# syghmon/bridges-with-reinforcement-learning

Hardware: AMD Instinct MI355X
Metric: env-steps/sec (vectorised assembly_gym, tower_height=4) (higher is better)
Workload: dtype f64

## Files before the change

__graft_entry__.py:

```python
import os
import subprocess
import sys

ROOT = os.path.dirname(os.path.abspath(__file__))
PKG = os.path.join(ROOT, "bridges-with-reinforcement-learning_amd")
for p in (ROOT, PKG):
    if p not in sys.path:
        sys.path.insert(0, p)

HIPCC = os.environ.get("HIPCC", "/opt/rocm/bin/hipcc")
HIP_FLAGS = ["--offload-arch=gfx950", "-O3", "-ffp-contract=off", "-fPIC", "-shared", "-std=c++17"]


def build():
    from bridges_hip import abi
    src = os.path.join(PKG, "csrc", "api.hip")
    out = os.path.join(PKG, "bridges_hip", "libbridges_hip.so")
    want = abi.source_hash()
    if abi.library_stamp(out) != want:
        tmp = out + ".tmp"
        subprocess.check_call([HIPCC, *HIP_FLAGS, f'-DBRIDGES_SRC_HASH="{want}"', src, "-o", tmp])
        os.replace(tmp, out)
        assert abi.library_stamp(out) == want, "the built library does not carry its source stamp"
    oracle_mk = os.path.join(ROOT, "oracle", "Makefile")
    if os.path.exists(oracle_mk):
        subprocess.check_call(["make", "-s", "-C", os.path.join(ROOT, "oracle")])
    import bridges_hip
    L = abi.lib()
    for sym in abi.EXPORTED_SYMBOLS:
        getattr(L, sym)


def smoke():
    import numpy as np
    import torch
    from bridges_hip.shapes import load_urdf
    from bridges_hip.vec_env import VecAssemblyGym
    from oracle.env import OracleGym, OracleLockstep, bridge_setup, policy_draw

    assert torch.cuda.is_available(), "smoke() needs cuda:0"
    E, seed = 8, 5
    setup = bridge_setup(num_stories=2)
    vec = VecAssemblyGym(E, [load_urdf("shapes/trapezoid.urdf")], setup["obstacles"], setup["targets"],
                         max_steps=10, seed=seed)
    oracles = [OracleLockstep(OracleGym(**setup, max_steps=10)) for _ in range(E)]
    counters = [0] * E
    for it in range(6):
        vec.select_random()
        outs = []
        for e, o in enumerate(oracles):
            def pick(nv, e=e):
                r = policy_draw(seed, e, counters[e]) % nv
                counters[e] += 1
                return r
            outs.append(o.lockstep(pick))
        vec.step()
        torch.cuda.synchronize()
        fl = {k: v.cpu().numpy() for k, v in vec.flags().items()}
        for e, out in enumerate(outs):
            if out["valid_step"]:
                assert bool(fl["stable_frozen"][e]) == out["stable_frozen"]
                assert bool(fl["stable_unfrozen"][e]) == out["stable_unfrozen"]
                assert bool(fl["done"][e]) == out["done"]
        off = vec.cand_offset.cpu().numpy()
        mask = vec.cand_mask.cpu().numpy()
        for e, o in enumerate(oracles):
            A = len(o.cand["actions"])
            assert np.array_equal(mask[off[e]:off[e] + A].astype(bool), o.cand["mask"])
    print("smoke ok: 6 lock-steps x 8 envs bit-identical to the oracle")


if __name__ == "__main__":
    {"build": build, "smoke": smoke}[sys.argv[1] if len(sys.argv) > 1 else "build"]()
```

bridges-with-reinforcement-learning_amd/csrc/api.hip:

```cpp
#include <hip/hip_runtime.h>
#include <cstdio>
#include <cstdlib>
#include <cstring>
#include <new>

#include "env_kernels.hip"
#include "ops_kernels.hip"
#include "dqn_kernels.hip"
#include "mlp_kernels.hip"
#include "conv_kernels.hip"
#include "conv_train_kernels.hip"
#include "replay_kernels.hip"
#include "hindsight_kernels.hip"
#include "fork_kernels.hip"
#include "beam_kernels.hip"
#include "soft_target_kernels.hip"
#include "munchausen_kernels.hip"

using namespace bridges;

static thread_local char g_err[512] = "";

static int fail_hip(hipError_t e, const char* what) {
    snprintf(g_err, sizeof(g_err), "%s: %s", what, hipGetErrorString(e));
    return BRIDGES_E_HIP;
}
static int fail_arg(const char* what) {
    snprintf(g_err, sizeof(g_err), "bad argument: %s", what);
    return BRIDGES_E_ARG;
}
static int fail_arg(const char* who, const char* what) {
    snprintf(g_err, sizeof(g_err), "bad argument: %s: %s", who, what);
    return BRIDGES_E_ARG;
}
#define HIP_TRY(x)                                        \
    do {                                                  \
        hipError_t e_ = (x);                              \
        if (e_ != hipSuccess) return fail_hip(e_, #x);    \
    } while (0)

template <typename... P, typename... A>
static int launch(const char* name, void (*k)(P...), dim3 grid, dim3 block, size_t lds, void* stream, A... a) {
    hipLaunchKernelGGL(k, grid, block, lds, (hipStream_t)stream, a...);
    const hipError_t e = hipGetLastError();
    return e == hipSuccess ? BRIDGES_OK : fail_hip(e, name);
}

template <typename... T>
static bool aligned(uintptr_t bytes, const T*... p) {
    return ((((uintptr_t)p) | ... | (uintptr_t)0) & (bytes - 1)) == 0;
}

static int64_t ceil_div(int64_t a, int64_t b) { return (a + b - 1) / b; }

static int64_t clamp_grid(int64_t blocks, int64_t limit) {
    if (blocks < 1) blocks = 1;
    return blocks > limit ? limit : blocks;
}

static int grid_for_waves(int64_t n_items) { return (int)clamp_grid(ceil_div(n_items, 4), 2048); }

static int up2_splits(int64_t tiles, int* tps) {
    int per = (int)((tiles + 255) / 256);
    if (per < 1) per = 1;
    *tps = per;
    return (int)((tiles + per - 1) / per);
}

typedef void (*c3_fn)(const float*, const float*, const float*, const float*, const float*, float*, int, int, int, int, int);
template <int W, int CH>
static c3_fn c3_epilogue(int mode) {
    if (mode == C3_EPI_BIAS_RELU) return k_c3<W, CH, C3_EPI_BIAS_RELU>;
    if (mode == C3_EPI_MASK) return k_c3<W, CH, C3_EPI_MASK>;
    return k_c3<W, CH, C3_EPI_RAW>;
}
template <int W>
static c3_fn c3_kernel(int c_in, int mode) { return c_in <= 4 ? c3_epilogue<W, 4>(mode) : c3_epilogue<W, 16>(mode); }

struct bridges_gate {
    hipEvent_t last;
};

struct bridges_env {
    bridges_gate* gate;
    hipEvent_t raster_done;
    DevCtx ctx;
    TaskTable* tt_dev;
    int32_t* h_total;
    int max_blocks;
    int max_faces;
    hipEvent_t* ev_start;
    hipEvent_t* ev_stop;
    int ev_cap, ev_used;
    bool has_tasks;
    bridges_task_buffers tasks;
    const float* fixed_reward_map;
    const double* fixed_reward_prefix;
    bridges_task_family family;
    const uint64_t* family_thr;
};

static void clear_family(bridges_env* env) {
    memset(&env->family, 0, sizeof(env->family));
    env->family_thr = nullptr;
}

static long long candidate_estimate(const bridges_env* env) {
    long long est = (long long)(*(volatile int32_t*)env->h_total);
    if (est < env->ctx.E) est = env->ctx.E;
    return est + est / 32 + 64;
}

extern "C" {

const char* bridges_last_error(void) { return g_err; }

#ifndef BRIDGES_SRC_HASH
#define BRIDGES_SRC_HASH "unstamped"
#endif
const char* bridges_source_hash(void) { return "BRIDGES_SRC_HASH=" BRIDGES_SRC_HASH; }

int bridges_device_count(void) {
    int n = 0;
    if (hipGetDeviceCount(&n) != hipSuccess) return 0;
    return n;
}

int bridges_env_create(const bridges_task* t, const bridges_env_buffers* buf, bridges_env** out) {
    if (!t || !buf || !out) return fail_arg("null");
    if (t->n_envs <= 0) return fail_arg("n_envs");
    if (t->max_blocks <= 0 || t->max_blocks > BRIDGES_MAX_BLOCKS) return fail_arg("max_blocks > BRIDGES_MAX_BLOCKS");
    if (t->n_shapes <= 0 || t->n_shapes > 8) return fail_arg("n_shapes");
    if (t->n_groups <= 0 || t->n_groups > BRIDGES_MAX_GROUPS) return fail_arg("n_groups");
    if (t->n_ground < 0 || t->n_ground > 32 || t->n_offsets <= 0 || t->n_offsets > 8) return fail_arg("n_ground/n_offsets");
    if (t->n_targets < 0 || t->n_targets > BRIDGES_MAX_TARGETS) return fail_arg("n_targets");
    if (t->a_max <= 0) return fail_arg("a_max");
    if (t->img_size != 0 && (t->img_size < 2 || t->img_size > BRIDGES_IMG)) return fail_arg("img_size must be 0 (= 64) or 2..64");
    if (t->debug != 0) return fail_arg("debug must be 0");
    if (!buf->reward_prefix) return fail_arg("reward_prefix (float64 row prefix sums of reward_map) not given");
    if (buf->lp_ws_stride < (int64_t)BRIDGES_LP_WS_DOUBLES) return fail_arg("lp_ws_stride < BRIDGES_LP_WS_DOUBLES");
    static_assert(BRIDGES_LP_WS_DOUBLES == WARM_WS_DOUBLES, "header and device code disagree on the persistent tableau size");
    static_assert(BRIDGES_LP_SNAP_DOUBLES == WARM_HDR_DOUBLES + WARM_HALF, "header and device code disagree on the snapshot size");
    if (buf->lp_snap && buf->lp_snap_stride < (int64_t)BRIDGES_LP_SNAP_DOUBLES) return fail_arg("lp_snap_stride < BRIDGES_LP_SNAP_DOUBLES");
    for (int g = 0; g < t->n_groups; ++g) {
        if (t->group_shape[g] < 0 || t->group_shape[g] >= t->n_shapes) return fail_arg("group_shape");
        if (t->group_face[g] < 0 || t->group_face[g] >= t->shapes[t->group_shape[g]].nv) return fail_arg("group_face");
    }
    for (int s = 0; s < t->n_shapes; ++s)
        if (t->shapes[s].nv < 3 || t->shapes[s].nv > BRIDGES_MAX_VERTS) return fail_arg("shape nv");
    int ndev = 0;
    if (hipGetDeviceCount(&ndev) != hipSuccess || ndev == 0) {
        snprintf(g_err, sizeof(g_err), "no HIP device");
        return BRIDGES_E_NODEV;
    }
    bridges_env* env = new (std::nothrow) bridges_env();
    if (!env) return fail_arg("oom");
    TaskTable* host = new (std::nothrow) TaskTable();
    if (!host) { delete env; return fail_arg("oom"); }
    memset(host, 0, sizeof(TaskTable));
    memcpy(host->shapes, t->shapes, sizeof(bridges_shape) * t->n_shapes);
    memcpy(host->x_ground, t->x_ground, sizeof(double) * t->n_ground);
    memcpy(host->offsets, t->offsets, sizeof(double) * t->n_offsets);
    const int img = t->img_size ? t->img_size : IMG;
    for (int i = 0; i < IMG; ++i) {
        host->grid_x[i] = t->grid_x[i < img ? i : img - 1];
        host->grid_y[i] = t->grid_y[i < img ? i : img - 1];
    }
    hipError_t e = hipMalloc((void**)&env->tt_dev, sizeof(TaskTable));
    if (e == hipSuccess) e = hipMemcpy(env->tt_dev, host, sizeof(TaskTable), hipMemcpyHostToDevice);
    delete host;
    if (e != hipSuccess) { delete env; return fail_hip(e, "task table upload"); }
    DevCtx& c = env->ctx;
    memset(&c, 0, sizeof(c));
    c.b = *buf;
    c.tt = env->tt_dev;
    c.E = t->n_envs; c.K = t->max_blocks; c.max_steps = t->max_steps; c.a_max = t->a_max;
    c.n_groups = t->n_groups; c.n_ground = t->n_ground; c.n_offsets = t->n_offsets; c.n_targets = t->n_targets;
    memcpy(c.group_shape, t->group_shape, sizeof(c.group_shape));
    memcpy(c.group_face, t->group_face, sizeof(c.group_face));
    c.mu = t->mu; c.density = t->density; c.floor_hw = t->floor_half_width; c.floor_depth = t->floor_depth;
    c.xlim0 = t->xlim[0]; c.xlim1 = t->xlim[1]; c.ylim0 = t->ylim[0]; c.ylim1 = t->ylim[1];
    memcpy(c.targets, t->targets, sizeof(c.targets));
    c.seed = t->seed;
    c.debug = t->debug;
    c.env_id_base = t->env_id_base;
    c.n_shapes = t->n_shapes;
    c.img = img;
    env->ev_start = env->ev_stop = nullptr;
    env->ev_cap = env->ev_used = 0;
    env->gate = nullptr;
    env->raster_done = nullptr;
    env->has_tasks = false;
    memset(&env->tasks, 0, sizeof(env->tasks));
    clear_family(env);
    env->fixed_reward_map = buf->reward_map;
    env->fixed_reward_prefix = buf->reward_prefix;
    e = hipHostMalloc((void**)&env->h_total, sizeof(int32_t), hipHostMallocMapped | hipHostMallocCoherent);
    if (e == hipSuccess) e = hipHostGetDevicePointer((void**)&c.h_total, env->h_total, 0);
    if (e != hipSuccess) { (void)hipFree(env->tt_dev); delete env; return fail_hip(e, "hipHostMalloc"); }
    *env->h_total = t->n_envs * 64;
    env->max_blocks = 1 << 22;
    env->max_faces = 0;
    for (int g = 0; g < t->n_groups; ++g) {
        const int nv = t->shapes[t->group_shape[g]].nv;
        if (nv > env->max_faces) env->max_faces = nv;
    }
    *out = env;
    return BRIDGES_OK;
}

static void free_events(bridges_env* env) {
    for (int i = 0; i < env->ev_cap; ++i) {
        (void)hipEventDestroy(env->ev_start[i]);
        (void)hipEventDestroy(env->ev_stop[i]);
    }
    delete[] env->ev_start;
    delete[] env->ev_stop;
    env->ev_start = env->ev_stop = nullptr;
    env->ev_cap = env->ev_used = 0;
}

int bridges_env_destroy(bridges_env* env) {
    if (!env) return BRIDGES_OK;
    free_events(env);
    if (env->raster_done) (void)hipEventDestroy(env->raster_done);
    (void)hipFree(env->tt_dev);
    (void)hipHostFree(env->h_total);
    delete env;
    return BRIDGES_OK;
}

int bridges_gate_create(bridges_gate** out) {
    if (!out) return fail_arg("gate_create");
    bridges_gate* g = new (std::nothrow) bridges_gate();
    if (!g) return fail_arg("oom");
    g->last = nullptr;
    *out = g;
    return BRIDGES_OK;
}

int bridges_gate_destroy(bridges_gate* gate) {
    delete gate;
    return BRIDGES_OK;
}

int bridges_env_set_gate(bridges_env* env, bridges_gate* gate) {
    if (!env) return fail_arg("set_gate");
    if (gate && !env->raster_done) HIP_TRY(hipEventCreateWithFlags(&env->raster_done, hipEventDisableTiming));
    env->gate = gate;
    return BRIDGES_OK;
}

int bridges_env_timing_begin(bridges_env* env, int32_t max_launches) {
    if (!env || max_launches <= 0 || max_launches > (1 << 16)) return fail_arg("timing_begin");
    free_events(env);
    env->ev_start = new (std::nothrow) hipEvent_t[max_launches];
    env->ev_stop = new (std::nothrow) hipEvent_t[max_launches];
    if (!env->ev_start || !env->ev_stop) {
        delete[] env->ev_start;
        delete[] env->ev_stop;
        env->ev_start = env->ev_stop = nullptr;
        return fail_arg("oom");
    }
    for (int i = 0; i < max_launches; ++i) {
        HIP_TRY(hipEventCreate(&env->ev_start[i]));
        HIP_TRY(hipEventCreate(&env->ev_stop[i]));
        env->ev_cap = i + 1;
    }
    env->ev_used = 0;
    return BRIDGES_OK;
}

int bridges_env_timing_end(bridges_env* env, double* raster_ms_total, int32_t* n_launches) {
    if (!env || !raster_ms_total || !n_launches) return fail_arg("timing_end");
    double total = 0.0;
    for (int i = 0; i < env->ev_used; ++i) {
        HIP_TRY(hipEventSynchronize(env->ev_stop[i]));
        float ms = 0.f;
        HIP_TRY(hipEventElapsedTime(&ms, env->ev_start[i], env->ev_stop[i]));
        total += ms;
    }
    *raster_ms_total = total;
    *n_launches = env->ev_used;
    free_events(env);
    return BRIDGES_OK;
}

static int refresh(bridges_env* env, hipStream_t s, int after_step) {
    const DevCtx& c = env->ctx;
    if (int rc = launch("k_scan", k_scan, dim3(1), dim3(SCAN_THREADS), 0, s, c, after_step)) return rc;
    if (int rc = launch("k_enumerate", k_enumerate, dim3(c.E), dim3(WAVE), 0, s, c)) return rc;
    const long long items_est = candidate_estimate(env) + c.E;
    long long rblocks = ceil_div(items_est, 4);
    if (rblocks > env->max_blocks) rblocks = env->max_blocks;
    const bool timed = env->ev_cap > 0 && env->ev_used < env->ev_cap;
    if (env->gate && env->gate->last) HIP_TRY(hipStreamWaitEvent(s, env->gate->last, 0));
    if (timed) HIP_TRY(hipEventRecord(env->ev_start[env->ev_used], s));
    if (!env->has_tasks) {
        if (int rc = launch("k_raster", env->max_faces <= 4 ? k_raster<4> : k_raster<MAXV>, dim3((unsigned)rblocks), dim3(256), 0, s, c))
            return rc;
    } else if (env->tasks.n_obstacles == 0) {
        if (int rc = launch("k_raster (per-env tables)", env->max_faces <= 4 ? k_raster<4, true> : k_raster<MAXV, true>,
                            dim3((unsigned)rblocks), dim3(256), 0, s, c))
            return rc;
    } else if (int rc = launch("k_raster (per-env tables and obstacles)", env->max_faces <= 4 ? k_raster<4, true, const uint64_t*> : k_raster<MAXV, true, const uint64_t*>,
                               dim3((unsigned)rblocks), dim3(256), 0, s, c, (const uint64_t*)env->tasks.env_obstacle_bits)) {
        return rc;
    }
    if (timed) { HIP_TRY(hipEventRecord(env->ev_stop[env->ev_used], s)); env->ev_used++; }
// ... 1525 lines not shown
```

bridges-with-reinforcement-learning_amd/csrc/bridges_device.h:

```cpp
#pragma once
#include <hip/hip_runtime.h>
#include <stdint.h>
#include "../../include/bridges_hip.h"

#define WAVE 64
#define MAXV BRIDGES_MAX_VERTS
#define MAXK BRIDGES_MAX_BLOCKS
#define MAXIF BRIDGES_MAX_INTERFACES
#define IMG BRIDGES_IMG

namespace bridges {

struct Frame2 {
    double cx, cz, tx, tz, nx, nz;
};

__device__ __forceinline__ Frame2 edge_frame(double ax, double az, double bx, double bz) {
    Frame2 f;
    f.cx = (ax + bx) * 0.5;
    f.cz = (az + bz) * 0.5;
    double dx = bx - ax;
    double dz = bz - az;
    double L = sqrt(dx * dx + dz * dz);
    f.tx = dx / L;
// ... 38 lines not shown

__device__ __forceinline__ uint64_t shfl_u64(uint64_t v, int src) {
    uint32_t lo = (uint32_t)v, hi = (uint32_t)(v >> 32);
    lo = __shfl(lo, src, WAVE);
    hi = __shfl(hi, src, WAVE);
    return ((uint64_t)hi << 32) | lo;
}

#define DPP_QUAD_XOR1 0xB1
#define DPP_QUAD_XOR2 0x4E
#define DPP_ROW_HALF_MIRROR 0x141
#define DPP_ROW_MIRROR 0x140
#define DPP_ROW_BCAST15 0x142
#define DPP_ROW_BCAST31 0x143

template <int CTRL, int ROW_MASK>
__device__ __forceinline__ int dpp_i(int old, int x) {
    return __builtin_amdgcn_update_dpp(old, x, CTRL, ROW_MASK, 0xF, false);
}
template <int CTRL, int ROW_MASK>
__device__ __forceinline__ double dpp_d(double old, double x) {
    int lo = dpp_i<CTRL, ROW_MASK>(__double2loint(old), __double2loint(x));
    int hi = dpp_i<CTRL, ROW_MASK>(__double2hiint(old), __double2hiint(x));
    return __hiloint2double(hi, lo);
}
__device__ __forceinline__ double readlane_d(double v, int lane_uniform) {
    int lo = __builtin_amdgcn_readlane(__double2loint(v), lane_uniform);
    int hi = __builtin_amdgcn_readlane(__double2hiint(v), lane_uniform);
    return __hiloint2double(hi, lo);
}
#define WAVE_REDUCE_D(OP, IDENT_OLD)                                                   \
    v = OP(v, dpp_d<DPP_QUAD_XOR1, 0xF>(v, v));                                        \
    v = OP(v, dpp_d<DPP_QUAD_XOR2, 0xF>(v, v));                                        \
    v = OP(v, dpp_d<DPP_ROW_HALF_MIRROR, 0xF>(v, v));                                  \
    v = OP(v, dpp_d<DPP_ROW_MIRROR, 0xF>(v, v));                                       \
    v = OP(v, dpp_d<DPP_ROW_BCAST15, 0xA>(IDENT_OLD, v));                              \
    v = OP(v, dpp_d<DPP_ROW_BCAST31, 0xC>(IDENT_OLD, v));                              \
    return readlane_d(v, 63);

__device__ __forceinline__ double add_d_(double a, double b) { return a + b; }
__device__ __forceinline__ double min_raw_d(double a, double b) { double r; asm volatile("v_min_f64 %0, %1, %2\n\ts_nop 1" : "=v"(r) : "v"(a), "v"(b)); return r; }
__device__ __forceinline__ double max_raw_d(double a, double b) { double r; asm volatile("v_max_f64 %0, %1, %2\n\ts_nop 1" : "=v"(r) : "v"(a), "v"(b)); return r; }
__device__ __forceinline__ double wave_sum_d(double v) { WAVE_REDUCE_D(add_d_, 0.0) }
__device__ __forceinline__ double wave_min_d(double v) { WAVE_REDUCE_D(min_raw_d, v) }
__device__ __forceinline__ double wave_max_d(double v) { WAVE_REDUCE_D(max_raw_d, v) }
__device__ __forceinline__ int wave_min_i(int v) {
    v = min(v, dpp_i<DPP_QUAD_XOR1, 0xF>(v, v));
    v = min(v, dpp_i<DPP_QUAD_XOR2, 0xF>(v, v));
    v = min(v, dpp_i<DPP_ROW_HALF_MIRROR, 0xF>(v, v));
    v = min(v, dpp_i<DPP_ROW_MIRROR, 0xF>(v, v));
    v = min(v, dpp_i<DPP_ROW_BCAST15, 0xA>(v, v));
    v = min(v, dpp_i<DPP_ROW_BCAST31, 0xC>(v, v));
    return __builtin_amdgcn_readlane(v, 63);
}

struct Adam {
    float step_size, bc2_sqrt, w1, w2, beta2, eps;
    __device__ __forceinline__ Adam(double lr, double beta1_d, double beta2_d, double eps_d, double t) {
        step_size = (float)(lr / (1.0 - pow(beta1_d, t)));
        bc2_sqrt = (float)sqrt(1.0 - pow(beta2_d, t));
        w1 = (float)(1.0 - beta1_d); w2 = (float)(1.0 - beta2_d); beta2 = (float)beta2_d; eps = (float)eps_d;
    }
    __device__ __forceinline__ void apply(float& p, float g, float& m, float& v) const {
        m = m + (g - m) * w1;
        v = beta2 * v + w2 * g * g;
        p = p - step_size * m / (sqrtf(v) / bc2_sqrt + eps);
    }
    __device__ __forceinline__ void apply(float4& p, const float4& g, float4& m, float4& v) const {
        apply(p.x, g.x, m.x, v.x);
        apply(p.y, g.y, m.y, v.y);
        apply(p.z, g.z, m.z, v.z);
        apply(p.w, g.w, m.w, v.w);
    }
};

struct TaskTable {
    bridges_shape shapes[8];
    double x_ground[32];
    double offsets[8];
    double grid_x[IMG];
    double grid_y[IMG];
};

struct DevCtx {
    bridges_env_buffers b;
    const TaskTable* tt;
    int32_t* h_total;
    int32_t E, K, max_steps, a_max, n_groups, n_ground, n_offsets, n_targets;
    int32_t debug, env_id_base;
    int32_t n_shapes, img;
    int32_t group_shape[BRIDGES_MAX_GROUPS];
    int32_t group_face[BRIDGES_MAX_GROUPS];
    double mu, density, floor_hw, floor_depth;
    double xlim0, xlim1, ylim0, ylim1;
    double targets[BRIDGES_MAX_TARGETS][3];
    uint64_t seed;
};

enum { F_VALID = 0, F_STABLE_FROZEN, F_STABLE_UNFROZEN, F_TERMINATED, F_TRUNCATED, F_DONE, F_NO_ACTIONS, F_LP_ERROR };
enum { ST_SUM_CAND = 0, ST_SUM_BLOCKS, ST_ENV_STEPS, ST_RESET_ONLY, ST_LP_ERRORS, ST_IF_OVERFLOW, ST_LOCKSTEPS, ST_SUM_VALID, ST_WARM_RESOLVED, ST_CAND_OVERFLOW };

}
```

bridges-with-reinforcement-learning_amd/csrc/env_kernels.hip:

```cpp
#include "bridges_device.h"
#include "rbe_device.h"

namespace bridges {

__device__ inline void reset_env(const DevCtx& c, int e, int lane) {
    c.b.state_bits[(size_t)e * IMG + lane] = 0ull;
    if (lane < c.K) c.b.blk_occ[(size_t)e * c.K + lane] = 0;
    if (lane == 0) {
        c.b.n_blocks[e] = 0;
        c.b.n_if[e] = 0;
        c.b.targets_left[e] = (c.n_targets >= 32) ? 0xffffffffu : ((1u << c.n_targets) - 1u);
        c.b.needs_reset[e] = 0;
    }
}

__device__ inline int count_candidates(const DevCtx& c, int e, int nb, int lane) {
    int nfree = 0;
    for (int i0 = 0; i0 < nb * MAXV; i0 += WAVE) {
        int i = i0 + lane;
        bool fr = false;
        if (i < nb * MAXV) {
            int b = i / MAXV, f = i % MAXV;
            int nv = c.tt->shapes[c.b.blk_shape[(size_t)e * c.K + b]].nv;
            fr = f < nv && !((c.b.blk_occ[(size_t)e * c.K + b] >> f) & 1);
// ... 268 lines not shown
    if (t == 0) carry_s = 0;
    __syncthreads();
    unsigned long long acc[8] = {0, 0, 0, 0, 0, 0, 0, 0};
    for (int base0 = 0; base0 < c.E; base0 += SCAN_THREADS * SCAN_BATCH) {
        int v[SCAN_BATCH], nbk[SCAN_BATCH], nval[SCAN_BATCH];
        uint64_t fl8[SCAN_BATCH];
#pragma unroll
        for (int u = 0; u < SCAN_BATCH; ++u) {
            const int i = base0 + u * SCAN_THREADS + t;
            const bool in = i < c.E;
            v[u] = in ? c.b.n_cand[i] : 0;
            nbk[u] = in ? c.b.n_blocks[i] : 0;
            nval[u] = (in && after_step) ? c.b.n_valid[i] : 0;
            fl8[u] = (in && after_step) ? *reinterpret_cast<const uint64_t*>(c.b.step_flags + (size_t)i * 8) : 0ull;
        }
#pragma unroll
        for (int u = 0; u < SCAN_BATCH; ++u) {
            const int base = base0 + u * SCAN_THREADS;
            if (base >= c.E) break;
            const int i = base + t;
            if (i < c.E) {
                if (v[u] > c.a_max) {
                    v[u] = c.a_max;
                    c.b.n_cand[i] = c.a_max;
                    c.b.step_flags[(size_t)i * 8 + F_LP_ERROR] |= 8;
                    acc[7] += 1;
                }
                acc[0] += (unsigned long long)nbk[u];
                if (after_step) {
                    const unsigned valid = (unsigned)(fl8[u] >> (8 * F_VALID)) & 0xffu;
                    const unsigned lperr = (unsigned)(fl8[u] >> (8 * F_LP_ERROR)) & 0xffu;
                    acc[1] += valid ? 1 : 0;
                    acc[2] += valid ? 0 : 1;
                    acc[3] += (lperr & 1) ? 1 : 0;
                    acc[4] += (lperr & 2) ? 1 : 0;
                    acc[5] += (unsigned long long)nval[u];
                    acc[6] += (lperr & 4) ? 1 : 0;
                }
            }
            int incl = v[u];
#pragma unroll
            for (int o = 1; o < WAVE; o <<= 1) {
                int up = __shfl_up(incl, o, WAVE);
                if (lane >= o) incl += up;
            }
            if (lane == WAVE - 1) wave_tot[wv] = incl;
            __syncthreads();
            int wbase = 0;
            for (int k = 0; k < wv; ++k) wbase += wave_tot[k];
            const int carry = carry_s;
            if (i < c.E) c.b.cand_offset[i] = carry + wbase + incl - v[u];
            __syncthreads();
            if (t == SCAN_THREADS - 1) carry_s = carry + wbase + incl;
            __syncthreads();
        }
    }
#pragma unroll
    for (int k = 0; k < 8; ++k) {
        unsigned long long x = acc[k];
#pragma unroll
        for (int o = 32; o > 0; o >>= 1) x += __shfl_xor(x, o, WAVE);
        if (lane == 0) red[wv][k] = x;
    }
    __syncthreads();
    if (t == 0) {
        unsigned long long tot[8] = {0, 0, 0, 0, 0, 0, 0, 0};
        for (int w = 0; w < SCAN_WAVES; ++w)
            for (int k = 0; k < 8; ++k) tot[k] += red[w][k];
        c.b.cand_offset[c.E] = carry_s;
        if (c.h_total) *c.h_total = carry_s;
        c.b.stats[ST_SUM_CAND] += (uint64_t)carry_s;
        c.b.stats[ST_SUM_BLOCKS] += tot[0];
        c.b.stats[ST_ENV_STEPS] += tot[1];
        c.b.stats[ST_RESET_ONLY] += tot[2];
        c.b.stats[ST_LP_ERRORS] += tot[3];
        c.b.stats[ST_IF_OVERFLOW] += tot[4];
        c.b.stats[ST_SUM_VALID] += tot[5];
        c.b.stats[ST_WARM_RESOLVED] += tot[6];
        c.b.stats[ST_CAND_OVERFLOW] += tot[7];
        c.b.stats[ST_LOCKSTEPS] += 1;
    }
}

__global__ __launch_bounds__(WAVE) void k_enumerate(DevCtx c) {
    __shared__ uint8_t free_b[MAXK * MAXV], free_f[MAXK * MAXV];
    __shared__ bridges_shape sh_l[8];
    __shared__ double verts_l[MAXK * MAXV * 2];
    __shared__ int32_t shape_l[MAXK], occ_l[MAXK];
    __shared__ double xg_l[32], offs_l[8];
    __builtin_amdgcn_s_setprio(3);
    const int e = blockIdx.x, lane = threadIdx.x;
    const int K = c.K;
    if (lane < 32) xg_l[lane] = c.tt->x_ground[lane];
    if (lane < 8) offs_l[lane] = c.tt->offsets[lane];
    const int nb = c.b.n_blocks[e];
    const int ncand = c.b.n_cand[e];
    const size_t off = (size_t)c.b.cand_offset[e];
    {
        const double* src = reinterpret_cast<const double*>(c.tt->shapes);
        double* dst = reinterpret_cast<double*>(sh_l);
        const int nd = c.n_shapes * (int)(sizeof(bridges_shape) / 8);
        for (int i = lane; i < nd; i += WAVE) dst[i] = src[i];
        const double* vg = c.b.blk_verts + (size_t)e * K * MAXV * 2;
        for (int i = lane; i < nb * MAXV * 2; i += WAVE) verts_l[i] = vg[i];
        if (lane < K) { shape_l[lane] = c.b.blk_shape[(size_t)e * K + lane]; occ_l[lane] = c.b.blk_occ[(size_t)e * K + lane]; }
    }
    __syncthreads();
    const bridges_shape* shapes = sh_l;
    const int32_t* shape_id = shape_l;
    const double* verts = verts_l;
    int nfree = 0;
    for (int i0 = 0; i0 < nb * MAXV; i0 += WAVE) {
        int i = i0 + lane;
        bool fr = false;
        int b = i / MAXV, f = i % MAXV;
        if (i < nb * MAXV) {
            int nv = shapes[shape_id[b]].nv;
            fr = f < nv && !((occ_l[b] >> f) & 1);
        }
        uint64_t bal = __ballot(fr);
        if (fr) {
            int idx = nfree + __popcll(bal & ((1ull << lane) - 1ull));
            free_b[idx] = (uint8_t)b;
            free_f[idx] = (uint8_t)f;
        }
        nfree += __popcll(bal);
    }
    __syncthreads();
    const int gsize = c.n_ground + nfree * c.n_offsets;
    for (int a = lane; a < ncand; a += WAVE) {
        int grp = a / gsize, slot = a % gsize;
        int sh = c.group_shape[grp], fc = c.group_face[grp];
        int tb = -1, tf = 0;
        double ox;
        Frame2 f1;
        if (slot < c.n_ground) {
            ox = xg_l[slot];
            f1.cx = 0.0; f1.cz = 0.0; f1.tx = 1.0; f1.tz = 0.0; f1.nx = 0.0; f1.nz = 1.0;
        } else {
            int k = (slot - c.n_ground) / c.n_offsets;
            ox = offs_l[(slot - c.n_ground) % c.n_offsets];
            tb = free_b[k]; tf = free_f[k];
            const bridges_shape& st = shapes[shape_id[tb]];
            const double* v = verts + (size_t)tb * MAXV * 2;
            f1 = edge_frame(v[2 * st.fa[tf]], v[2 * st.fa[tf] + 1], v[2 * st.fb[tf]], v[2 * st.fb[tf] + 1]);
        }
        const bridges_shape& sn = shapes[sh];
        double px, pz, cs, sn_;
        align_place(f1, sn.fcx[fc], sn.fcz[fc], sn.fnx[fc], sn.fnz[fc], ox, 0.0, px, pz, cs, sn_);
        const size_t ci = off + a;
        bool inb = true;
        const double eps = 1e-6;
        double wx[MAXV], wz[MAXV];
#pragma unroll
        for (int i = 0; i < MAXV; ++i) {
            wx[i] = 0.0; wz[i] = 0.0;
            if (i < sn.nv) {
                double rx, rz;
                rot2(sn.vx[i], sn.vz[i], cs, sn_, rx, rz);
                wx[i] = px + rx; wz[i] = pz + rz;
                if (wx[i] < c.xlim0 - eps || wx[i] > c.xlim1 + eps || wz[i] < c.ylim0 - eps || wz[i] > c.ylim1 + eps) inb = false;
                if (wz[i] < -eps) inb = false;
            }
            c.b.cand_verts[ci * MAXV * 2 + 2 * i] = wx[i];
            c.b.cand_verts[ci * MAXV * 2 + 2 * i + 1] = wz[i];
        }
        {
#define PICK6(v, k) ((k) == 5 ? v[5] : (k) == 4 ? v[4] : (k) == 3 ? v[3] : (k) == 2 ? v[2] : (k) == 1 ? v[1] : v[0])
#pragma unroll
            for (int f = 0; f < MAXV; ++f) {
                double o0 = 0.0, o1 = 0.0, o2 = 0.0, o3 = 0.0;
                if (f < sn.nv) {
                    const int ia = sn.fa[f], ib = sn.fb[f];
                    const double ax = PICK6(wx, ia), az = PICK6(wz, ia), bx = PICK6(wx, ib), bz = PICK6(wz, ib);
                    Frame2 fr = edge_frame(ax, az, bx, bz);
                    o0 = fr.cx; o1 = fr.cz; o2 = fr.nx; o3 = fr.nz;
                }
                double2* dst = reinterpret_cast<double2*>(c.b.cand_frames + (ci * MAXV + f) * 4);
                dst[0] = make_double2(o0, o1);
                dst[1] = make_double2(o2, o3);
            }
#undef PICK6
            c.b.cand_rows[ci * 2 + 0] = (sn.nv << 16) | ((inb ? 1 : 0) << 24);
            c.b.cand_rows[ci * 2 + 1] = e;
        }
        c.b.cand_pose[ci * 4 + 0] = px; c.b.cand_pose[ci * 4 + 1] = pz;
        c.b.cand_pose[ci * 4 + 2] = cs; c.b.cand_pose[ci * 4 + 3] = sn_;
        c.b.cand_desc[ci * 4 + 0] = tb; c.b.cand_desc[ci * 4 + 1] = tf;
        c.b.cand_desc[ci * 4 + 2] = sh; c.b.cand_desc[ci * 4 + 3] = fc;
        c.b.cand_ox[ci] = ox;
        c.b.cand_inb[ci] = inb;
        c.b.cand_env[ci] = e;
    }
}

__device__ __forceinline__ void write_f32_image(float* img, uint64_t rowbits, int lane, int32_t* nz = nullptr) {
    const int sub = lane >> 4, col4 = (lane & 15) * 4;
    const uint64_t nonzero_rows = __ballot(rowbits != 0ull);
    if (nz) {
        uint64_t t = nonzero_rows | (nonzero_rows >> 1);
        t = (t | (t >> 2)) & 0x1111111111111111ull;
        uint32_t now = 0u;
#pragma unroll
        for (int g = 0; g < IMG / 4; ++g) now |= (uint32_t)((t >> (4 * g)) & 1ull) << g;
        uint32_t need = (uint32_t)__builtin_amdgcn_readfirstlane(*nz) | now;
        if (lane == 0) *nz = (int32_t)now;
        while (need) {
            const int g = __builtin_ctz(need);
            need &= need - 1u;
            uint32_t nib = 0u;
            if ((now >> g) & 1u) {
                uint64_t m = shfl_u64(rowbits, 4 * g + sub);
                nib = (uint32_t)(m >> col4) & 0xFu;
            }
            float4 v;
            v.x = (nib & 1u) ? 1.f : 0.f;
            v.y = (nib & 2u) ? 1.f : 0.f;
            v.z = (nib & 4u) ? 1.f : 0.f;
            v.w = (nib & 8u) ? 1.f : 0.f;
            *reinterpret_cast<float4*>(img + (size_t)(4 * g + sub) * IMG + col4) = v;
        }
        return;
    }
#pragma unroll
    for (int r0 = 0; r0 < IMG; r0 += 4) {
        uint32_t nib = 0u;
        if ((nonzero_rows >> r0) & 0xFull) {
            uint64_t m = shfl_u64(rowbits, r0 + sub);
            nib = (uint32_t)(m >> col4) & 0xFu;
        }
        float4 v;
        v.x = (nib & 1u) ? 1.f : 0.f;
        v.y = (nib & 2u) ? 1.f : 0.f;
        v.z = (nib & 4u) ? 1.f : 0.f;
        v.w = (nib & 8u) ? 1.f : 0.f;
        *reinterpret_cast<float4*>(img + (size_t)(r0 + sub) * IMG + col4) = v;
    }
}

__device__ __forceinline__ uint64_t low_mask64(int n) { return n >= 64 ? ~0ull : ((1ull << n) - 1ull); }

template <int NF, int F0 = 0>
__device__ __forceinline__ uint64_t raster_rows(double fr0, double fr1, double fr2, double fr3, int n_img, double X, double Y,
                                                int lane) {
    int alo[NF], ahi[NF], pos[NF];
    double t[NF];
    bool rev[NF];
#pragma unroll
    for (int f = 0; f < NF; ++f) {
        const double cxf = readlane_d(fr0, F0 + f), czf = readlane_d(fr1, F0 + f), nxf = readlane_d(fr2, F0 + f), nzf = readlane_d(fr3, F0 + f);
        const double a = (X - cxf) * nxf;
        t[f] = -((Y - czf) * nzf);
        alo[f] = __double2loint(a);
        ahi[f] = __double2hiint(a);
        rev[f] = nxf < 0.0;
        pos[f] = 0;
    }
#define RASTER_PROBE(S_, INC_)                                                                                          \
    _Pragma("unroll") for (int f = 0; f < NF; ++f) {                                                                    \
        const int j = pos[f] + (S_);                                                                                    \
        const int src = rev[f] ? 63 - j : j;                                                                            \
        const double av = __hiloint2double(__shfl(ahi[f], src, WAVE), __shfl(alo[f], src, WAVE));                       \
        if (av <= t[f]) pos[f] += (INC_);                                                                               \
    }
    RASTER_PROBE(31, 32) RASTER_PROBE(15, 16) RASTER_PROBE(7, 8) RASTER_PROBE(3, 4) RASTER_PROBE(1, 2) RASTER_PROBE(0, 1)
    RASTER_PROBE(0, 1)
#undef RASTER_PROBE
    uint64_t bits = low_mask64(n_img);
#pragma unroll
    for (int f = 0; f < NF; ++f) {
        const uint64_t run = low_mask64(pos[f]);
        bits &= rev[f] ? (pos[f] ? ~low_mask64(64 - pos[f]) : 0ull) : run;
    }
    return lane < n_img ? bits : 0ull;
}

__device__ __forceinline__ uint64_t raster_rows6(double fr0, double fr1, double fr2, double fr3, int n_img, double X, double Y, int lane) {
    return raster_rows<3, 0>(fr0, fr1, fr2, fr3, n_img, X, Y, lane) & raster_rows<3, 3>(fr0, fr1, fr2, fr3, n_img, X, Y, lane);
}

__device__ __forceinline__ uint64_t raster_rows_nv(double fr0, double fr1, double fr2, double fr3, int nv, int n_img, double X,
                                                   double Y, int lane) {
    return nv <= 4 ? raster_rows<4>(fr0, fr1, fr2, fr3, n_img, X, Y, lane) : raster_rows6(fr0, fr1, fr2, fr3, n_img, X, Y, lane);
}

__device__ __forceinline__ void raster_reward_fetch(uint64_t rowbits, const double* prefix, int lane, double& p_hi, double& p_lo) {
    p_hi = 0.0; p_lo = 0.0;
    if (rowbits) {
        const int lo = __builtin_ctzll(rowbits), hi = 64 - __builtin_clzll(rowbits);
        const double* p = prefix + lane * (IMG + 1);
        p_hi = p[hi]; p_lo = p[lo];
    }
}
__device__ __forceinline__ double raster_reward_sum(double p_hi, double p_lo) { return wave_sum_d(p_hi - p_lo); }

__device__ __forceinline__ uint64_t raster_outline(const double* v , int nv, const int32_t* fa,
                                                   const int32_t* fb, const double* gx, const double* gy, int size, int lane) {
    double cx = 0.0, cz = 0.0, nx = 0.0, nz = 0.0;
    if (lane < nv) {
        Frame2 fr = edge_frame(v[2 * fa[lane]], v[2 * fa[lane] + 1], v[2 * fb[lane]], v[2 * fb[lane] + 1]);
        cx = fr.cx; cz = fr.cz; nx = fr.nx; nz = fr.nz;
    }
    const int g = lane < size ? lane : size - 1;
    return raster_rows_nv(cx, cz, nx, nz, nv, size, gx[g], gy[g], lane);
}

__device__ __forceinline__ const uint64_t* raster_env_obst() { return nullptr; }
__device__ __forceinline__ const uint64_t* raster_env_obst(const uint64_t* p) { return p; }
template <int NF, bool PER_ENV = false, typename... ENV_OBST_ARG>
__global__ __launch_bounds__(256) void k_raster(DevCtx c, ENV_OBST_ARG... env_obst_arg) {
    constexpr bool ENV_OBST = sizeof...(ENV_OBST_ARG) == 1;
    const uint64_t* env_obst = raster_env_obst(env_obst_arg...);
    (void)env_obst;
    const int lane = threadIdx.x & (WAVE - 1);
    const int wave = (blockIdx.x * blockDim.x + threadIdx.x) / WAVE;
    const int nwaves = (gridDim.x * blockDim.x) / WAVE;
    const int total = c.b.cand_offset[c.E];
    const int items = total + (c.b.state_raster ? c.E : 0);
    const double X = c.tt->grid_x[lane], Y = c.tt->grid_y[lane];
    const uint64_t obst = ENV_OBST ? 0ull : c.b.obstacle_bits[lane];
    for (int itv = wave; itv < items; itv += nwaves) {
        const int it = __builtin_amdgcn_readfirstlane(itv);
        if (it < total) {
            const size_t ci = (size_t)it;
            const int meta = c.b.cand_rows[ci * 2];
            const int e = c.b.cand_rows[ci * 2 + 1];
            const int nv = (meta >> 16) & 0xff;
            const bool inb = (meta >> 24) & 1;
            (void)nv;
            double fr0 = 0.0, fr1 = 0.0, fr2 = 0.0, fr3 = 0.0;
            if (lane < MAXV) {
                const double2* p = reinterpret_cast<const double2*>(c.b.cand_frames + (ci * MAXV + lane) * 4);
                const double2 a = p[0], b = p[1];
                fr0 = a.x; fr1 = a.y; fr2 = b.x; fr3 = b.y;
            }
            const uint64_t occ = c.b.state_bits[(size_t)e * IMG + lane] | (ENV_OBST ? env_obst[(size_t)e * IMG + lane] : obst);
            const uint64_t bits = (NF == 4 || nv <= 4) ? raster_rows<4>(fr0, fr1, fr2, fr3, c.img, X, Y, lane)
                                                       : raster_rows6(fr0, fr1, fr2, fr3, c.img, X, Y, lane);
            const bool overlap = __ballot((bits & occ) != 0ull) != 0ull;
            double p_hi, p_lo;
            raster_reward_fetch(bits, PER_ENV ? c.b.reward_prefix + (size_t)e * (IMG * (IMG + 1)) : c.b.reward_prefix, lane, p_hi, p_lo);
            c.b.cand_bits[ci * IMG + lane] = bits;
            if (c.b.cand_raster)
                write_f32_image(c.b.cand_raster + ci * IMG * IMG, bits, lane, c.b.cand_raster_nz ? c.b.cand_raster_nz + ci : nullptr);
            const double lin = raster_reward_sum(p_hi, p_lo);
            if (lane == 0) {
                c.b.cand_lin[ci] = (float)lin;
                c.b.cand_mask[ci] = (uint8_t)(inb && !overlap);
            }
        } else {
            const int e = it - total;
            write_f32_image(c.b.state_raster + (size_t)e * IMG * IMG, c.b.state_bits[(size_t)e * IMG + lane], lane,
                            c.b.state_raster_nz ? c.b.state_raster_nz + e : nullptr);
        }
    }
}


enum { TASK_LOAD = 0, TASK_RESET = 1, TASK_STEP = 2 };
#define TASK_SALT 0x7461736B5F726E67ull
#define OBST_SALT 0x6F6273745F726E67ull
#define TASK_ROW (IMG + 1)
#define TASK_WAVES 4
#define TASK_THREADS (TASK_WAVES * WAVE)
#define TASK_ROWS_IN_FLIGHT 4
#define TASK_KZ_PAD 16
#define TASK_KZ (TASK_KZ_PAD + BRIDGES_GAUSS_TAPS + 16)
static_assert(IMG - 1 - BRIDGES_GAUSS_TAPS / 2 <= TASK_KZ_PAD && IMG - 1 + BRIDGES_GAUSS_TAPS / 2 < BRIDGES_GAUSS_TAPS + 16,
              "every tap index of a 64 x 64 canvas must fall into the padded table");
static_assert(IMG % (TASK_WAVES * TASK_ROWS_IN_FLIGHT) == 0, "map rows are dealt to the waves in batches");
#define FAMI_SALT 0x66616D695F726E67ull
__device__ __forceinline__ int family_class(uint64_t seed, uint32_t gid, uint32_t ep, int n_lo, int n_hi, const uint64_t* thr) {
    const uint64_t h0 = splitmix64((((seed & 0xFFFFFFFFull) << 32) | gid) ^ FAMI_SALT);
    const uint64_t h1 = splitmix64(h0 ^ (uint64_t)ep);
    const uint64_t r = splitmix64(h1);
    const uint64_t u = r >> 32;
    const int C = n_hi - n_lo + 1;
    if (!thr) return n_lo + (int)((u * (uint64_t)C) >> 32);
    int n = n_lo;
    for (int k = 0; k < C - 1; ++k) n += u >= thr[k] ? 1 : 0;
    return n;
}
__device__ __forceinline__ bridges_task_family task_family() { return bridges_task_family{}; }
__device__ __forceinline__ bridges_task_family task_family(const bridges_task_family& f) { return f; }
__device__ __forceinline__ bridges_task_family task_family(const bridges_task_family& f, const uint64_t*) { return f; }
__device__ __forceinline__ const uint64_t* task_thresholds() { return nullptr; }
__device__ __forceinline__ const uint64_t* task_thresholds(const bridges_task_family&) { return nullptr; }
__device__ __forceinline__ const uint64_t* task_thresholds(const bridges_task_family&, const uint64_t* thr) { return thr; }
template <bool STORE_MAP>
__device__ __forceinline__ void task_map_prefix(const uint64_t bits, const uint64_t* tb_l, const float* kz, float* map_l, double* pre_l,
                                                const int S, const int lane, const int wv, float* map_g) {
    const uint64_t nzrows = __ballot(bits != 0ull);
    const int half = BRIDGES_GAUSS_TAPS / 2;
    for (int b = 0; b < IMG / (TASK_WAVES * TASK_ROWS_IN_FLIGHT); ++b) {
        const int y0 = (wv * (IMG / TASK_WAVES)) + b * TASK_ROWS_IN_FLIGHT;
        double acc[TASK_ROWS_IN_FLIGHT];
#pragma unroll
        for (int r = 0; r < TASK_ROWS_IN_FLIGHT; ++r) acc[r] = 0.0;
        uint64_t rows = y0 < S ? nzrows : 0ull;
        while (rows) {
            const int py = __builtin_ctzll(rows);
            rows &= rows - 1ull;
            float ki[TASK_ROWS_IN_FLIGHT];
#pragma unroll
            for (int r = 0; r < TASK_ROWS_IN_FLIGHT; ++r) ki[r] = kz[py - (y0 + r) + half + TASK_KZ_PAD];
            const uint64_t row = tb_l[py];
            uint64_t m = ((uint64_t)(uint32_t)__builtin_amdgcn_readfirstlane((int)(uint32_t)(row >> 32)) << 32) |
                         (uint32_t)__builtin_amdgcn_readfirstlane((int)(uint32_t)row);
            while (m) {
                const int pxl = __builtin_ctzll(m);
                m &= m - 1ull;
                const float kx = kz[pxl - lane + half + TASK_KZ_PAD];
#pragma unroll
                for (int r = 0; r < TASK_ROWS_IN_FLIGHT; ++r) {
                    const float prod = ki[r] * kx;
                    acc[r] = acc[r] + (double)prod;
                }
            }
        }
#pragma unroll
        for (int r = 0; r < TASK_ROWS_IN_FLIGHT; ++r) {
            const int y = y0 + r;
            const float v = (lane < S && y < S) ? (float)acc[r] : 0.f;
            map_l[y * TASK_ROW + lane] = v;
            if constexpr (STORE_MAP) map_g[y * IMG + lane] = v;
        }
    }
    __syncthreads();
    if (wv == 0) {
        double run = 0.0;
        pre_l[lane * TASK_ROW] = 0.0;
        for (int x = 0; x < IMG; ++x) {
            run = run + (double)map_l[lane * TASK_ROW + x];
            pre_l[lane * TASK_ROW + x + 1] = run;
        }
    }
    __syncthreads();
}
// ... 428 lines not shown
```

Baseline: 4.669 million.

## Precompute ground-slot candidate placements and rasters into a device table at env creation

Ground-placed candidates depend only on group and ground slot, not on env state, so their pose, vertices, frames and raster bits are computed once into a GroundTable when the env is created. Enumeration copies from the table instead of recomputing, and the raster kernel loads the precomputed bits (flagged via the low 16 bits of cand_rows) instead of rasterising. A build-time check on VGPR, scratch and LDS use of the raster kernels is also added. The cost is extra device memory, extra copy traffic, and a new branch in the raster loop.

```diff
diff --git a/__graft_entry__.py b/__graft_entry__.py
--- a/__graft_entry__.py
+++ b/__graft_entry__.py
@@ -1,4 +1,5 @@
 import os
+import re
 import subprocess
 import sys
 
@@ -12,6 +13,26 @@
 HIP_FLAGS = ["--offload-arch=gfx950", "-O3", "-ffp-contract=off", "-fPIC", "-shared", "-std=c++17"]
 
 
+def raster_footprints(remarks):
+    found, name = {}, None
+    for line in remarks.splitlines():
+        m = re.search(r"remark:\s+Function Name: (\S+)", line)
+        if m:
+            name = m.group(1) if "8k_rasterI" in m.group(1) else None
+            continue
+        m = re.search(r"remark:\s+(VGPRs|ScratchSize|LDS Size)[^:]*: (\d+)", line)
+        if m and name:
+            found.setdefault(name, {})[m.group(1)] = int(m.group(2))
+    return found
+
+
+def check_raster_footprint(remarks):
+    found = raster_footprints(remarks)
+    assert len(found) == 6, f"expected the six k_raster instantiations in the compiler's remarks, found {sorted(found)}"
+    for name, use in sorted(found.items()):
+        assert use["VGPRs"] <= 64 and use["ScratchSize"] == 0 and use["LDS Size"] == 0, (name, use)
+
+
 def build():
     from bridges_hip import abi
     src = os.path.join(PKG, "csrc", "api.hip")
@@ -19,7 +40,12 @@
     want = abi.source_hash()
     if abi.library_stamp(out) != want:
         tmp = out + ".tmp"
-        subprocess.check_call([HIPCC, *HIP_FLAGS, f'-DBRIDGES_SRC_HASH="{want}"', src, "-o", tmp])
+        res = subprocess.run([HIPCC, *HIP_FLAGS, "-Rpass-analysis=kernel-resource-usage", f'-DBRIDGES_SRC_HASH="{want}"', src, "-o", tmp],
+                             stderr=subprocess.PIPE, text=True)
+        if res.returncode != 0:
+            sys.stderr.write(res.stderr)
+            raise subprocess.CalledProcessError(res.returncode, res.args)
+        check_raster_footprint(res.stderr)
         os.replace(tmp, out)
         assert abi.library_stamp(out) == want, "the built library does not carry its source stamp"
     oracle_mk = os.path.join(ROOT, "oracle", "Makefile")
diff --git a/bridges-with-reinforcement-learning_amd/csrc/api.hip b/bridges-with-reinforcement-learning_amd/csrc/api.hip
--- a/bridges-with-reinforcement-learning_amd/csrc/api.hip
+++ b/bridges-with-reinforcement-learning_amd/csrc/api.hip
@@ -86,6 +86,7 @@
     hipEvent_t raster_done;
     DevCtx ctx;
     TaskTable* tt_dev;
+    GroundTable* gt_dev;
     int32_t* h_total;
     int max_blocks;
     int max_faces;
@@ -198,6 +199,20 @@
     e = hipHostMalloc((void**)&env->h_total, sizeof(int32_t), hipHostMallocMapped | hipHostMallocCoherent);
     if (e == hipSuccess) e = hipHostGetDevicePointer((void**)&c.h_total, env->h_total, 0);
     if (e != hipSuccess) { (void)hipFree(env->tt_dev); delete env; return fail_hip(e, "hipHostMalloc"); }
+    e = hipMalloc((void**)&env->gt_dev, sizeof(GroundTable));
+    c.gt = env->gt_dev;
+    if (e == hipSuccess && c.n_ground > 0) {
+        hipLaunchKernelGGL(k_ground_table, dim3(c.n_groups * c.n_ground), dim3(WAVE), 0, (hipStream_t)0, c, env->gt_dev);
+        e = hipGetLastError();
+        if (e == hipSuccess) e = hipDeviceSynchronize();
+    }
+    if (e != hipSuccess) {
+        (void)hipFree(env->gt_dev);
+        (void)hipFree(env->tt_dev);
+        (void)hipHostFree(env->h_total);
+        delete env;
+        return fail_hip(e, "k_ground_table");
+    }
     *env->h_total = t->n_envs * 64;
     env->max_blocks = 1 << 22;
     env->max_faces = 0;
@@ -225,6 +240,7 @@
     free_events(env);
     if (env->raster_done) (void)hipEventDestroy(env->raster_done);
     (void)hipFree(env->tt_dev);
+    (void)hipFree(env->gt_dev);
     (void)hipHostFree(env->h_total);
     delete env;
     return BRIDGES_OK;
diff --git a/bridges-with-reinforcement-learning_amd/csrc/bridges_device.h b/bridges-with-reinforcement-learning_amd/csrc/bridges_device.h
--- a/bridges-with-reinforcement-learning_amd/csrc/bridges_device.h
+++ b/bridges-with-reinforcement-learning_amd/csrc/bridges_device.h
@@ -144,6 +144,20 @@
     double grid_y[IMG];
 };
 
+#define GROUND_SLOTS 32
+#define GROUND_ENTRIES (BRIDGES_MAX_GROUPS * GROUND_SLOTS)
+static_assert(GROUND_ENTRIES + 1 < (1 << 16), "an entry index + 1 must fit the low 16 bits of cand_rows");
+struct GroundTable {
+    uint64_t bits[GROUND_ENTRIES][IMG];
+    double frames[GROUND_ENTRIES][MAXV * 4];
+    double verts[GROUND_ENTRIES][MAXV * 2];
+    double pose[GROUND_ENTRIES][4];
+    double ox[GROUND_ENTRIES];
+    int32_t desc[GROUND_ENTRIES][4];
+    int32_t nv[GROUND_ENTRIES];
+    uint8_t inb[GROUND_ENTRIES];
+};
+
 struct DevCtx {
     bridges_env_buffers b;
     const TaskTable* tt;
@@ -157,6 +171,7 @@
     double xlim0, xlim1, ylim0, ylim1;
     double targets[BRIDGES_MAX_TARGETS][3];
     uint64_t seed;
+    const GroundTable* gt;
 };
 
 enum { F_VALID = 0, F_STABLE_FROZEN, F_STABLE_UNFROZEN, F_TERMINATED, F_TRUNCATED, F_DONE, F_NO_ACTIONS, F_LP_ERROR };
diff --git a/bridges-with-reinforcement-learning_amd/csrc/env_kernels.hip b/bridges-with-reinforcement-learning_amd/csrc/env_kernels.hip
--- a/bridges-with-reinforcement-learning_amd/csrc/env_kernels.hip
+++ b/bridges-with-reinforcement-learning_amd/csrc/env_kernels.hip
@@ -374,16 +374,55 @@
     }
 }
 
+__device__ __forceinline__ bool place_candidate(const DevCtx& c, const bridges_shape& sn, int fc, const Frame2& f1, double ox,
+                                                double* pose, double* verts, double* frames) {
+    double px, pz, cs, sn_;
+    align_place(f1, sn.fcx[fc], sn.fcz[fc], sn.fnx[fc], sn.fnz[fc], ox, 0.0, px, pz, cs, sn_);
+    bool inb = true;
+    const double eps = 1e-6;
+    double wx[MAXV], wz[MAXV];
+#pragma unroll
+    for (int i = 0; i < MAXV; ++i) {
+        wx[i] = 0.0; wz[i] = 0.0;
+        if (i < sn.nv) {
+            double rx, rz;
+            rot2(sn.vx[i], sn.vz[i], cs, sn_, rx, rz);
+            wx[i] = px + rx; wz[i] = pz + rz;
+            if (wx[i] < c.xlim0 - eps || wx[i] > c.xlim1 + eps || wz[i] < c.ylim0 - eps || wz[i] > c.ylim1 + eps) inb = false;
+            if (wz[i] < -eps) inb = false;
+        }
+        verts[2 * i] = wx[i];
+        verts[2 * i + 1] = wz[i];
+    }
+#define PICK6(v, k) ((k) == 5 ? v[5] : (k) == 4 ? v[4] : (k) == 3 ? v[3] : (k) == 2 ? v[2] : (k) == 1 ? v[1] : v[0])
+#pragma unroll
+    for (int f = 0; f < MAXV; ++f) {
+        double o0 = 0.0, o1 = 0.0, o2 = 0.0, o3 = 0.0;
+        if (f < sn.nv) {
+            const int ia = sn.fa[f], ib = sn.fb[f];
+            const double ax = PICK6(wx, ia), az = PICK6(wz, ia), bx = PICK6(wx, ib), bz = PICK6(wz, ib);
+            Frame2 fr = edge_frame(ax, az, bx, bz);
+            o0 = fr.cx; o1 = fr.cz; o2 = fr.nx; o3 = fr.nz;
+        }
+        double2* dst = reinterpret_cast<double2*>(frames + f * 4);
+        dst[0] = make_double2(o0, o1);
+        dst[1] = make_double2(o2, o3);
+    }
+#undef PICK6
+    pose[0] = px; pose[1] = pz;
+    pose[2] = cs; pose[3] = sn_;
+    return inb;
+}
+
 __global__ __launch_bounds__(WAVE) void k_enumerate(DevCtx c) {
     __shared__ uint8_t free_b[MAXK * MAXV], free_f[MAXK * MAXV];
     __shared__ bridges_shape sh_l[8];
     __shared__ double verts_l[MAXK * MAXV * 2];
     __shared__ int32_t shape_l[MAXK], occ_l[MAXK];
-    __shared__ double xg_l[32], offs_l[8];
+    __shared__ double offs_l[8];
     __builtin_amdgcn_s_setprio(3);
     const int e = blockIdx.x, lane = threadIdx.x;
     const int K = c.K;
-    if (lane < 32) xg_l[lane] = c.tt->x_ground[lane];
     if (lane < 8) offs_l[lane] = c.tt->offsets[lane];
     const int nb = c.b.n_blocks[e];
     const int ncand = c.b.n_cand[e];
@@ -422,62 +461,41 @@
     const int gsize = c.n_ground + nfree * c.n_offsets;
     for (int a = lane; a < ncand; a += WAVE) {
         int grp = a / gsize, slot = a % gsize;
+        const size_t ci = off + a;
+        if (slot < c.n_ground) {
+            const GroundTable& g = *c.gt;
+            const int gi = grp * c.n_ground + slot;
+            const double2* pv = reinterpret_cast<const double2*>(g.verts[gi]);
+            double2* dv = reinterpret_cast<double2*>(c.b.cand_verts + ci * MAXV * 2);
+#pragma unroll
+            for (int i = 0; i < MAXV; ++i) dv[i] = pv[i];
+            const double2* pf = reinterpret_cast<const double2*>(g.frames[gi]);
+            double2* df = reinterpret_cast<double2*>(c.b.cand_frames + ci * MAXV * 4);
+#pragma unroll
+            for (int i = 0; i < MAXV * 2; ++i) df[i] = pf[i];
+            c.b.cand_rows[ci * 2 + 0] = g.nv[gi] | (gi + 1);
+            c.b.cand_rows[ci * 2 + 1] = e;
+            const double2* pp = reinterpret_cast<const double2*>(g.pose[gi]);
+            double2* dp = reinterpret_cast<double2*>(c.b.cand_pose + ci * 4);
+            dp[0] = pp[0]; dp[1] = pp[1];
+            *reinterpret_cast<int4*>(c.b.cand_desc + ci * 4) = *reinterpret_cast<const int4*>(g.desc[gi]);
+            c.b.cand_ox[ci] = g.ox[gi];
+            c.b.cand_inb[ci] = g.inb[gi];
+            c.b.cand_env[ci] = e;
+            continue;
+        }
         int sh = c.group_shape[grp], fc = c.group_face[grp];
-        int tb = -1, tf = 0;
-        double ox;
-        Frame2 f1;
-        if (slot < c.n_ground) {
-            ox = xg_l[slot];
-            f1.cx = 0.0; f1.cz = 0.0; f1.tx = 1.0; f1.tz = 0.0; f1.nx = 0.0; f1.nz = 1.0;
-        } else {
-            int k = (slot - c.n_ground) / c.n_offsets;
-            ox = offs_l[(slot - c.n_ground) % c.n_offsets];
-            tb = free_b[k]; tf = free_f[k];
-            const bridges_shape& st = shapes[shape_id[tb]];
-            const double* v = verts + (size_t)tb * MAXV * 2;
-            f1 = edge_frame(v[2 * st.fa[tf]], v[2 * st.fa[tf] + 1], v[2 * st.fb[tf]], v[2 * st.fb[tf] + 1]);
-        }
+        const int k = (slot - c.n_ground) / c.n_offsets;
+        const double ox = offs_l[(slot - c.n_ground) % c.n_offsets];
+        const int tb = free_b[k], tf = free_f[k];
+        const bridges_shape& st = shapes[shape_id[tb]];
+        const double* v = verts + (size_t)tb * MAXV * 2;
+        const Frame2 f1 = edge_frame(v[2 * st.fa[tf]], v[2 * st.fa[tf] + 1], v[2 * st.fb[tf]], v[2 * st.fb[tf] + 1]);
         const bridges_shape& sn = shapes[sh];
-        double px, pz, cs, sn_;
-        align_place(f1, sn.fcx[fc], sn.fcz[fc], sn.fnx[fc], sn.fnz[fc], ox, 0.0, px, pz, cs, sn_);
-        const size_t ci = off + a;
-        bool inb = true;
-        const double eps = 1e-6;
-        double wx[MAXV], wz[MAXV];
-#pragma unroll
-        for (int i = 0; i < MAXV; ++i) {
-            wx[i] = 0.0; wz[i] = 0.0;
-            if (i < sn.nv) {
-                double rx, rz;
-                rot2(sn.vx[i], sn.vz[i], cs, sn_, rx, rz);
-                wx[i] = px + rx; wz[i] = pz + rz;
-                if (wx[i] < c.xlim0 - eps || wx[i] > c.xlim1 + eps || wz[i] < c.ylim0 - eps || wz[i] > c.ylim1 + eps) inb = false;
-                if (wz[i] < -eps) inb = false;
-            }
-            c.b.cand_verts[ci * MAXV * 2 + 2 * i] = wx[i];
-            c.b.cand_verts[ci * MAXV * 2 + 2 * i + 1] = wz[i];
-        }
-        {
-#define PICK6(v, k) ((k) == 5 ? v[5] : (k) == 4 ? v[4] : (k) == 3 ? v[3] : (k) == 2 ? v[2] : (k) == 1 ? v[1] : v[0])
-#pragma unroll
-            for (int f = 0; f < MAXV; ++f) {
-                double o0 = 0.0, o1 = 0.0, o2 = 0.0, o3 = 0.0;
-                if (f < sn.nv) {
-                    const int ia = sn.fa[f], ib = sn.fb[f];
-                    const double ax = PICK6(wx, ia), az = PICK6(wz, ia), bx = PICK6(wx, ib), bz = PICK6(wz, ib);
-                    Frame2 fr = edge_frame(ax, az, bx, bz);
-                    o0 = fr.cx; o1 = fr.cz; o2 = fr.nx; o3 = fr.nz;
-                }
-                double2* dst = reinterpret_cast<double2*>(c.b.cand_frames + (ci * MAXV + f) * 4);
-                dst[0] = make_double2(o0, o1);
-                dst[1] = make_double2(o2, o3);
-            }
-#undef PICK6
-            c.b.cand_rows[ci * 2 + 0] = (sn.nv << 16) | ((inb ? 1 : 0) << 24);
-            c.b.cand_rows[ci * 2 + 1] = e;
-        }
-        c.b.cand_pose[ci * 4 + 0] = px; c.b.cand_pose[ci * 4 + 1] = pz;
-        c.b.cand_pose[ci * 4 + 2] = cs; c.b.cand_pose[ci * 4 + 3] = sn_;
+        const bool inb = place_candidate(c, sn, fc, f1, ox, c.b.cand_pose + ci * 4, c.b.cand_verts + ci * MAXV * 2,
+                                         c.b.cand_frames + ci * MAXV * 4);
+        c.b.cand_rows[ci * 2 + 0] = (sn.nv << 16) | ((inb ? 1 : 0) << 24);
+        c.b.cand_rows[ci * 2 + 1] = e;
         c.b.cand_desc[ci * 4 + 0] = tb; c.b.cand_desc[ci * 4 + 1] = tf;
         c.b.cand_desc[ci * 4 + 2] = sh; c.b.cand_desc[ci * 4 + 3] = fc;
         c.b.cand_ox[ci] = ox;
@@ -620,6 +638,25 @@
             const int nv = (meta >> 16) & 0xff;
             const bool inb = (meta >> 24) & 1;
             (void)nv;
+            const int gi = meta & 0xffff;
+            if (gi) {
+                uintptr_t rows = reinterpret_cast<uintptr_t>(c.gt->bits[gi - 1]);
+                asm volatile("" : "+s"(rows));
+                const uint64_t bits = reinterpret_cast<const __attribute__((address_space(1))) uint64_t*>(rows)[lane];
+                const uint64_t occ = c.b.state_bits[(size_t)e * IMG + lane] | (ENV_OBST ? env_obst[(size_t)e * IMG + lane] : obst);
+                double p_hi, p_lo;
+                raster_reward_fetch(bits, PER_ENV ? c.b.reward_prefix + (size_t)e * (IMG * (IMG + 1)) : c.b.reward_prefix, lane, p_hi, p_lo);
+                c.b.cand_bits[ci * IMG + lane] = bits;
+                if (c.b.cand_raster)
+                    write_f32_image(c.b.cand_raster + ci * IMG * IMG, bits, lane, c.b.cand_raster_nz ? c.b.cand_raster_nz + ci : nullptr);
+                const bool overlap = __ballot((bits & occ) != 0ull) != 0ull;
+                const double lin = raster_reward_sum(p_hi, p_lo);
+                if (lane == 0) {
+                    c.b.cand_lin[ci] = (float)lin;
+                    c.b.cand_mask[ci] = (uint8_t)(inb && !overlap);
+                }
+                continue;
+            }
             double fr0 = 0.0, fr1 = 0.0, fr2 = 0.0, fr3 = 0.0;
             if (lane < MAXV) {
                 const double2* p = reinterpret_cast<const double2*>(c.b.cand_frames + (ci * MAXV + lane) * 4);
@@ -646,6 +683,30 @@
                             c.b.state_raster_nz ? c.b.state_raster_nz + e : nullptr);
         }
     }
+}
+
+__global__ __launch_bounds__(WAVE) void k_ground_table(DevCtx c, GroundTable* gt) {
+    __shared__ __attribute__((aligned(16))) double frames_l[MAXV * 4];
+    const int gi = blockIdx.x, lane = threadIdx.x;
+    const int grp = gi / c.n_ground, slot = gi % c.n_ground;
+    const int sh = c.group_shape[grp], fc = c.group_face[grp];
+    const bridges_shape& sn = c.tt->shapes[sh];
+    if (lane == 0) {
+        const double ox = c.tt->x_ground[slot];
+        Frame2 f1;
+        f1.cx = 0.0; f1.cz = 0.0; f1.tx = 1.0; f1.tz = 0.0; f1.nx = 0.0; f1.nz = 1.0;
+        const bool inb = place_candidate(c, sn, fc, f1, ox, gt->pose[gi], gt->verts[gi], frames_l);
+        gt->desc[gi][0] = -1; gt->desc[gi][1] = 0;
+        gt->desc[gi][2] = sh; gt->desc[gi][3] = fc;
+        gt->ox[gi] = ox;
+        gt->inb[gi] = inb;
+        gt->nv[gi] = (sn.nv << 16) | ((inb ? 1 : 0) << 24);
+    }
+    __syncthreads();
+    if (lane < MAXV * 4) gt->frames[gi][lane] = frames_l[lane];
+    double fr0 = 0.0, fr1 = 0.0, fr2 = 0.0, fr3 = 0.0;
+    if (lane < MAXV) { fr0 = frames_l[lane * 4]; fr1 = frames_l[lane * 4 + 1]; fr2 = frames_l[lane * 4 + 2]; fr3 = frames_l[lane * 4 + 3]; }
+    gt->bits[gi][lane] = raster_rows_nv(fr0, fr1, fr2, fr3, sn.nv, c.img, c.tt->grid_x[lane], c.tt->grid_y[lane], lane);
 }
 
 
```

Measured after the change: 4.637 million. Within noise of the previous version (-0.7%).
